# bplaut/PyTorch-VAE

Measured on AMD Instinct MI355X. Metric: train images/sec (node) VanillaVAE 64×64 bs=64 at 1/2/4/8 GPU; ELBO match, higher is better.
Workload: dtype bf16; 1 GPU; VanillaVAE latent_dim=128 64x64 train step (fwd+ELBO+bwd+Adam); per_gpu_batch=64, global_batch=64, parallelism=dp1, graph=True, comm=none

## Files before the change

pytorch-vae_amd/csrc/vae_cgemm.hpp:

```cpp
#pragma once
#include "vae_igemm.hpp"

namespace vae {

template <int BM, int BN> struct CgWaves {
  static constexpr int WN = BN >= 2 * BM ? 4 : (BM >= 2 * BN ? 1 : 2);
  static constexpr int WM = 4 / WN;
  static constexpr int TM = BM / WM / 16, TN = BN / WN / 16;
  static_assert(TM >= 1 && TN >= 1, "wave tile below 16x16");
};

template <int XA>
__device__ __forceinline__ uint4 cg_xform(const uint32_t (&w)[4], const uint32_t (&y)[4], const Tab& t, int ch,
                                          float slope) {
  if constexpr (XA == VAE_X_NONE) {
    return uint4{w[0], w[1], w[2], w[3]};
  } else {
    uint4 o;
    uint32_t* op = reinterpret_cast<uint32_t*>(&o);
    f32x2 ab[4], bb[4], cb[4];
    if constexpr (XA != VAE_X_ACT) {
      const f32x4 a0 = tab4(t.a, ch), a1 = tab4(t.a, ch + 4);
      ab[0] = f32x2{a0[0], a0[1]}; ab[1] = f32x2{a0[2], a0[3]}; ab[2] = f32x2{a1[0], a1[1]}; ab[3] = f32x2{a1[2], a1[3]};
      {
// ... 40 lines not shown
template <int LOADS> constexpr int wg_stages() {
  return 20 / LOADS < 2 ? 2 : (20 / LOADS > 8 ? 8 : 20 / LOADS);
}

template <int BM, int BN, int BK, int NBUF = 2> struct CgSmem {
  static constexpr int LDK = BK + 8;
  static constexpr int LOOP = NBUF * (BM + BN) * LDK * 2;
  static constexpr int EPI = BM * (BN + 4) * 4;
  static constexpr int BYTES = LOOP > EPI ? LOOP : EPI;
};

template <int BM, int BN, int XA> constexpr int cg_waves_per_eu() {
  return (BM >= 128 && BN >= 128) ? 2 : ((BM == 64 && BN == 32 && XA == VAE_X_BN_DY) ? 3 : 1);
}

template <int BM, int BN, int BK, int AM, int XA, int EM, int OR>
__device__ __forceinline__ void cgemm_body(const GemmParams& p, const int bid, char* smem) {
  using WG = CgWaves<BM, BN>;
  constexpr int TM = WG::TM, TN = WG::TN, WTM = TM * 16, WTN = TN * 16;
  constexpr int LDK = CgSmem<BM, BN, BK>::LDK;
  constexpr int KC = BK / 8;
  constexpr int RPP = 256 / KC;
  constexpr int APT = (BM + RPP - 1) / RPP, BPT = (BN + RPP - 1) / RPP;
  constexpr bool DY = XA == VAE_X_BN_DY;
  constexpr int NSF = OR == 3 ? cg_ring_deep(APT * (DY ? 2 : 1) + BPT) : cg_stages<APT * (DY ? 2 : 1) + BPT>();
  constexpr int NS = OR == 2 ? (NSF < 2 ? NSF : 2) : NSF;
  constexpr int NBUF = OR == 2 ? 1 : 2;
  constexpr bool ABN = XA == VAE_X_BN_ACT || XA == VAE_X_BN_DY;
  static_assert(BM % RPP == 0 || BM < RPP, "A tile rows");
  static_assert(BN % RPP == 0 || BN < RPP, "B tile rows");

  extern __shared__ float tabs[];
  __bf16* As = reinterpret_cast<__bf16*>(smem);
  __bf16* Bs = As + NBUF * BM * LDK;

#ifdef VAE_PROBE
  unsigned long long clk[4] = {0, 0, 0, 0};
  const unsigned long long wall0 = threadIdx.x == 0 ? wall_clock64() : 0;
#endif
  PROBE_MARK(0);
  const int tid = threadIdx.x, lane = tid & 63;
  const int wave = __builtin_amdgcn_readfirstlane(tid >> 6);
  const int wm = wave / WG::WN, wn = wave % WG::WN;
  const int gm = (p.M + BM - 1) / BM, gn = (p.N + BN - 1) / BN, gz = p.nphase * p.ksplit;
  int tile;
  {
    const int nb = gm * gn * gz, b = bid;
    const int q = nb >> 3, r = nb & 7, x = b & 7, loc = b >> 3;
    tile = x * q + min(x, r) + loc;
  }
  int tn, tz, tmi;
  if (p.m_fast) { tmi = tile % gm; tz = (tile / gm) % gz; tn = tile / (gm * gz); }
  else { tn = tile % gn; tz = (tile / gn) % gz; tmi = tile / (gn * gz); }
  const int m0 = tmi * BM, n0 = tn * BN;
  const int phase = (p.nphase > 1) ? (int)(tz / p.ksplit) : 0;
  const int ks = tz - phase * p.ksplit;
  const bool first_block = tile == 0;

  const PhaseInfo pq = make_phase(p, phase);
  const int Kp = AM == A_CONVT ? pq.nth * pq.ntw * p.gc : p.K;
  const int ktiles = (Kp + BK - 1) / BK;
  const int kper = (ktiles + p.ksplit - 1) / p.ksplit;
  const int kt0 = ks * kper;
  const int kt1 = min(ktiles, kt0 + kper);
  const int kend = min(Kp, kt1 * BK);

  const int kc = tid % KC, r0 = tid / KC;
  const Src<__bf16> sa = make_src<__bf16>(p.a_ptr, p.a_bytes, p.a_xf);
  const rsrc_t rb = make_rsrc(p.b_ptr, p.b_bytes);
  RowOperand<__bf16, AM, true> ar[APT];
  int bbase[BPT];
  bool bok[BPT];
#pragma unroll
  for (int i = 0; i < APT; ++i) ar[i].init(p, m0 + r0 + i * RPP, p.M, phase, p.a_ld);
#pragma unroll
  for (int i = 0; i < BPT; ++i) {
    const int n = n0 + r0 + i * RPP;
    bok[i] = n < p.N && r0 + i * RPP < BN;
    bbase[i] = n * p.b_ld;
// ... 32 lines not shown
      const uint32_t off = (bok[i] && t.kin) ? (uint32_t)(bbase[i] + boff) * 2u : kOOB;
      bload<16>(rb, off, st.b[i]);
    }
  };

  const int ca = tab_stride(p.a_xf.channels), ce = tab_stride(p.epi_xf.channels);
  const Tab ta{tabs, tabs + ca, tabs + 2 * ca, nullptr, nullptr};
  float* tq = tabs + (ABN ? 3 * ca : 0);
  const Tab te{tq, tq + ce, nullptr, tq + 2 * ce, tq + 3 * ce};

  constexpr int TCH = 2;
  float tva[3][TCH], tve[4][TCH];
  const bool a_tab = ABN && p.a_xf.table != nullptr && p.a_xf.channels <= 256 * TCH;
  const bool e_tab = EM == E_BNBWD && p.epi_xf.kind == VAE_X_BN_ACT && p.epi_xf.table != nullptr &&
                     p.epi_xf.channels <= 256 * TCH;
  if (a_tab) {
    const int C = p.a_xf.channels;
#pragma unroll
    for (int j = 0; j < TCH; ++j) {
      const int ch = min(tid + 256 * j, C - 1);
#pragma unroll
      for (int q = 0; q < (DY ? 3 : 2); ++q) tva[q][j] = p.a_xf.table[q * C + ch];
    }
  }
  if (e_tab) {
    const int C = p.epi_xf.channels;
#pragma unroll
    for (int j = 0; j < TCH; ++j) {
      const int ch = min(tid + 256 * j, C - 1);
#pragma unroll
      for (int q = 0; q < 4; ++q) tve[q][j] = p.epi_xf.table[q * C + ch];
    }
  }
  TabPre<DY ? 4 : 2> pa;
  TabPre<2> pe;
  const bool a_pre = ABN && !a_tab && tab_pre_ok<XA>(p.a_xf);
  const bool e_pre = EM == E_BNBWD && !e_tab && tab_pre_ok<VAE_X_BN_ACT>(p.epi_xf);
  if (a_pre) tab_pre_load(p.a_xf, pa);
  if (e_pre) tab_pre_load(p.epi_xf, pe);
  Stage ring[NS];
#pragma unroll
  for (int u = 0; u < NS; ++u) {
    if (!OR || kt0 + u < kt1) issue(kt0 + u, ring[u]);
  }
  constexpr int EC = BN / 8, ERS = 256 / EC;
  constexpr int EPT = (BM + ERS - 1) / ERS;
  const int ec = tid % EC, er0 = tid / EC;
  const int col = n0 + ec * 8;
  const bool col_ok = col < p.N;
  uint32_t aux[EPT][4], res[EPT][4];
  int obase[EPT];
  bool rok[EPT];
  float bias[8];
  const bool has_res = p.residual != nullptr;
  constexpr bool EARLY = EPT <= 2 && cg_waves_per_eu<BM, BN, XA>() < 3;
  auto epi_loads = [&]() {
    const rsrc_t raux = epi_aux_rsrc<EM>(p);
    const rsrc_t rres = epi_res_rsrc<EM>(p);
    const bool loads = p.slab == nullptr;
#pragma unroll
    for (int i = 0; i < EPT; ++i) {
      const int rl = er0 + i * ERS, row = m0 + rl;
      rok[i] = rl < BM && row < p.M && col_ok;
      obase[i] = out_row_base(p, phase, rok[i] ? row : 0) + col;
      const uint32_t off = (rok[i] && loads) ? (uint32_t)obase[i] * 2u : kOOB;
      bload<16>(raux, off, aux[i]);
      if (EM == E_BNBWD && has_res) bload<16>(rres, off, res[i]);
      else res[i][0] = res[i][1] = res[i][2] = res[i][3] = 0u;
    }
#pragma unroll
    for (int e = 0; e < 8; ++e) bias[e] = 0.f;
    if (EM == E_STORE && p.bias && col_ok && loads) {
#pragma unroll
      for (int e = 0; e < 8; ++e) bias[e] = p.bias[col + e];
    }
  };
  if constexpr (EARLY) epi_loads();
  if (a_tab) {
    const int C = p.a_xf.channels;
#pragma unroll
    for (int j = 0; j < TCH; ++j) {
      const int ch = tid + 256 * j;
      if (ch < C) {
        ta.a[ch] = tva[0][j]; ta.b[ch] = tva[1][j];
        if (DY) ta.c[ch] = tva[2][j];
      }
    }
  } else if constexpr (ABN) {
    tab_fill_pre(p.a_xf, pa, a_pre, ta, false, first_block, reinterpret_cast<float*>(smem));
  }
  if constexpr (ABN) {
    if (tid < 8) { const int z = tab_pad(p.a_xf.channels) + tid; ta.a[z] = 0.f; ta.b[z] = 0.f; ta.c[z] = 0.f; }
  }
  if (e_tab) {
    const int C = p.epi_xf.channels;
#pragma unroll
    for (int j = 0; j < TCH; ++j) {
      const int ch = tid + 256 * j;
      if (ch < C) { te.a[ch] = tve[0][j]; te.b[ch] = tve[1][j]; te.p[ch] = tve[2][j]; te.q[ch] = tve[3][j]; }
    }
  } else if constexpr (EM == E_BNBWD) {
    tab_fill_pre(p.epi_xf, pe, e_pre, te, true, false, reinterpret_cast<float*>(smem));
  }
  __syncthreads();
  PROBE_MARK(1);

  f32x4 acc[TM][TN];
#pragma unroll
  for (int i = 0; i < TM; ++i)
#pragma unroll
    for (int j = 0; j < TN; ++j) acc[i][j] = f32x4{0.f, 0.f, 0.f, 0.f};

  auto store = [&](int buf, const Stage& st) {
    __bf16* ad = As + buf * BM * LDK + r0 * LDK + kc * 8;
#pragma unroll
    for (int i = 0; i < APT; ++i) {
      if (r0 + i * RPP < BM) {
// ... 20 lines not shown
      bf16x8 af[TM], bfr[TN];
#pragma unroll
      for (int i = 0; i < TM; ++i) af[i] = *reinterpret_cast<const bf16x8*>(a + i * 16 * LDK + 32 * kk);
#pragma unroll
      for (int j = 0; j < TN; ++j) bfr[j] = *reinterpret_cast<const bf16x8*>(b + j * 16 * LDK + 32 * kk);
#pragma unroll
      for (int i = 0; i < TM; ++i)
#pragma unroll
        for (int j = 0; j < TN; ++j) acc[i][j] = __builtin_amdgcn_mfma_f32_16x16x32_bf16(af[i], bfr[j], acc[i][j], 0, 0, 0);
    }
  };

  if constexpr (OR != 0) {
#pragma unroll
    for (int u = 0; u < NS; ++u) {
      if (kt0 + u < kt1) {
        if (NBUF == 1 && u > 0) __syncthreads();
        store(u & (NBUF - 1), ring[u]);
        __syncthreads();
        compute(u & (NBUF - 1));
      }
    }
  } else {
    int buf = 0;
    for (int kb = kt0; kb < kt1; kb += NS) {
#pragma unroll
      for (int u = 0; u < NS; ++u) {
        const bool live = kb + u < kt1;
        if (live) store(buf, ring[u]);
        __syncthreads();
        issue(kb + u + NS, ring[u]);
        if (live) compute(buf);
        buf ^= 1;
      }
    }
  }
  PROBE_MARK(2);
#ifdef VAE_PROBE
  struct ProbeEnd {
    unsigned long long* pr; unsigned long long* clk; unsigned long long w0;
    __device__ ~ProbeEnd() { PROBE_MARK(3); probe_write(pr, clk, w0); }
  } probe_end{p.probe, clk, wall0};
#endif

  __shared__ float fpart[CgWaves<BM, BN>::WM][2][BN];
  const bool frag_sums = EM == E_STORE && p.sum != nullptr && p.slab == nullptr;
  if (frag_sums) {
#pragma unroll
    for (int j = 0; j < TN; ++j) {
      float a1 = 0.f, a2 = 0.f;
#pragma unroll
      for (int i = 0; i < TM; ++i)
#pragma unroll
        for (int e = 0; e < 4; ++e) { a1 += acc[i][j][e]; a2 = fmaf(acc[i][j][e], acc[i][j][e], a2); }
      a1 += __shfl_xor(a1, 16); a2 += __shfl_xor(a2, 16);
      a1 += __shfl_xor(a1, 32); a2 += __shfl_xor(a2, 32);
      if (lane < 16) { fpart[wm][0][wn * WTN + j * 16 + lane] = a1; fpart[wm][1][wn * WTN + j * 16 + lane] = a2; }
    }
  }
  __syncthreads();
  float* Cs = reinterpret_cast<float*>(smem);
  constexpr int LDC = BN + 4;
  {
    const int rq = wm * WTM + 4 * (lane >> 4), cq = wn * WTN + (lane & 15);
#pragma unroll
    for (int i = 0; i < TM; ++i)
#pragma unroll
      for (int j = 0; j < TN; ++j)
#pragma unroll
        for (int e = 0; e < 4; ++e) Cs[(rq + i * 16 + e) * LDC + cq + j * 16] = acc[i][j][e];
  }
  __syncthreads();
  if (p.slab) {
    float* sl = p.slab + ((long)(phase * p.ksplit + ks) * p.M) * p.N;
#pragma unroll
    for (int i = 0; i < EPT; ++i) {
      const int rl = er0 + i * ERS, row = m0 + rl;
      if (rl < BM && row < p.M && col_ok) {
// ... 55 lines not shown
        }
        o[e] = g;
      }
    }
    uint32_t* pp = reinterpret_cast<uint32_t*>(&pk[i]);
#pragma unroll
    for (int e = 0; e < 4; ++e) {
      bf16x2 h;
      h[0] = (__bf16)o[2 * e];
      h[1] = (__bf16)o[2 * e + 1];
      pp[e] = *reinterpret_cast<uint32_t*>(&h);
    }
  }
  if (frag_sums) {
    for (int c = tid; c < BN; c += 256) {
      if (n0 + c < p.N) {
        float t1 = 0.f, t2 = 0.f;
#pragma unroll
        for (int w = 0; w < CgWaves<BM, BN>::WM; ++w) { t1 += fpart[w][0][c]; t2 += fpart[w][1][c]; }
        epi_flush_sums<EM>(p, bid, n0 + c, t1, t2);
      }
    }
  } else if (EM == E_BNBWD && epi_wants_sums<EM>(p)) {
    float* part = Cs;
#pragma unroll
    for (int m = EC; m < 64; m <<= 1) {
#pragma unroll
      for (int e = 0; e < 8; ++e) {
        s1[e] += __shfl_xor(s1[e], m);
        s2[e] += __shfl_xor(s2[e], m);
      }
    }
    __syncthreads();
    if (lane < EC) {
#pragma unroll
      for (int e = 0; e < 8; ++e) {
        part[(wave * 2) * BN + ec * 8 + e] = s1[e];
        part[(wave * 2 + 1) * BN + ec * 8 + e] = s2[e];
      }
    }
    __syncthreads();
    for (int c = tid; c < BN; c += 256) {
      if (n0 + c < p.N) {
        const float t1 = (part[0 * BN + c] + part[2 * BN + c]) + (part[4 * BN + c] + part[6 * BN + c]);
        const float t2 = (part[1 * BN + c] + part[3 * BN + c]) + (part[5 * BN + c] + part[7 * BN + c]);
        epi_flush_sums<EM>(p, bid, n0 + c, t1, t2);
      }
    }
  }
  __bf16* out = static_cast<__bf16*>(p.out);
#pragma unroll
  for (int i = 0; i < EPT; ++i)
    if (rok[i]) *reinterpret_cast<uint4*>(out + obase[i]) = pk[i];
}

template <int BM, int BN, int BK, int OR> constexpr int cg_nbuf() { return OR == 2 ? 1 : 2; }

template <int BM, int BN, int BK, int AM, int XA, int EM, int OR>
__global__ void __launch_bounds__(256) __attribute__((amdgpu_waves_per_eu(cg_waves_per_eu<BM, BN, XA>())))
cgemm_kernel(const GemmParams p) {
  kernarg_prefetch<sizeof(GemmParams)>();
  __shared__ __attribute__((aligned(16))) char smem[CgSmem<BM, BN, BK, cg_nbuf<BM, BN, BK, OR>()>::BYTES];
  cgemm_body<BM, BN, BK, AM, XA, EM, OR>(p, (int)blockIdx.x, smem);
}

}
```

pytorch-vae_amd/csrc/vae_common.hpp:

```cpp
#pragma once
#include <hip/hip_runtime.h>
#include <stdint.h>
#include <string.h>

#include "vaehip.h"

typedef float f32x4 __attribute__((ext_vector_type(4)));
typedef float f32x2 __attribute__((ext_vector_type(2)));
typedef __bf16 bf16x8 __attribute__((ext_vector_type(8)));
typedef __bf16 bf16x4 __attribute__((ext_vector_type(4)));
typedef __bf16 bf16x2 __attribute__((ext_vector_type(2)));

namespace vae {

void set_error(const char* fmt, ...);
int fail(int code, const char* fmt, ...);
int check_launch(const char* what);
int bn_finalize_launch(const vae_bn_args* a, hipStream_t stream);
constexpr int kRouteDeclined = 0x7fff0001;

inline int grid_for(long n, int per_block = 256, int max_blocks = 2048) {
  long b = (n + per_block - 1) / per_block;
  if (b < 1) b = 1;
  return (int)(b > max_blocks ? max_blocks : b);
// ... 310 lines not shown
__host__ __device__ inline int tab_stride(int c) { return tab_pad(c) + 8; }

__host__ __device__ inline bool bn_fast_ok(const vae_xform& x) {
  const int C = x.channels, R = x.reps > 1 ? x.reps : 1;
  if (C <= 0 || C > 512 || R * C > 1024 || (x.reps > 1 && x.rstride < C)) return false;
  return C <= 256 ? (256 % C == 0) : (C % 256 == 0);
}

template <int NS>
struct TabPre {
  float v[NS][4];
  float g, be, sh;
};

template <int NS>
__device__ __forceinline__ void tab_pre_load(const vae_xform& x, TabPre<NS>& q) {
  const int C = x.channels, R = x.reps > 1 ? x.reps : 1, tid = threadIdx.x;
  const long rs = x.reps > 1 ? x.rstride : 0;
  const int total = R * C;
  const float* arr[4] = {x.sum, x.sumsq, x.dgamma, x.dbeta};
#pragma unroll
  for (int k = 0; k < 4; ++k) {
    const int f = tid + 256 * k;
    const bool ok = f < total;
    const int r = ok ? f / C : 0, c = ok ? f - r * C : 0;
    const long o = (long)r * rs + c;
#pragma unroll
    for (int a = 0; a < NS; ++a) q.v[a][k] = ok ? arr[a][o] : 0.f;
  }
  const int ch = tid < C ? tid : C - 1;
  q.g = x.gamma[ch];
  q.be = x.beta[ch];
  q.sh = x.shift ? x.shift[ch] : 0.0f;
}

template <int NS>
__device__ __forceinline__ void tab_pre_finish(const vae_xform& x, const TabPre<NS>& q, Tab t, bool epi,
                                               bool update_running, float* scr) {
  const int C = x.channels, R = x.reps > 1 ? x.reps : 1, tid = threadIdx.x;
  float tot[2][4];
#pragma unroll
  for (int j = 0; j < 2; ++j)
#pragma unroll
    for (int a = 0; a < 4; ++a) tot[j][a] = 0.f;
  int nch = 1;
  if (C <= 256) {
#pragma unroll
    for (int a = 0; a < NS; ++a) scr[a * 256 + tid] = (q.v[a][0] + q.v[a][1]) + (q.v[a][2] + q.v[a][3]);
    __syncthreads();
    if (tid < C) {
#pragma unroll
      for (int a = 0; a < NS; ++a) {
        float acc = 0.f;
        for (int j = tid; j < 256; j += C) acc += scr[a * 256 + j];
        tot[0][a] = acc;
      }
    }
    __syncthreads();
    nch = tid < C ? 1 : 0;
  } else {
    const int per = C / 256;
#pragma unroll
    for (int j = 0; j < 2; ++j)
#pragma unroll
      for (int a = 0; a < NS; ++a) {
        float acc = 0.f;
#pragma unroll
        for (int k = 0; k < 4; ++k) acc += ((k % per) == j && k / per < R) ? q.v[a][k] : 0.f;
        tot[j][a] = acc;
      }
    nch = per;
  }
#pragma unroll
  for (int j = 0; j < 2; ++j) {
    if (j >= nch) break;
    const int ch = C <= 256 ? tid : tid + 256 * j;
    const float g = j == 0 ? q.g : x.gamma[ch];
    const float be = j == 0 ? q.be : x.beta[ch];
    const float sh = j == 0 ? q.sh : (x.shift ? x.shift[ch] : 0.0f);
    const BnMom mo = bn_mom(tot[j][0], tot[j][1], sh, x);
    if (x.kind == VAE_X_BN_ACT) {
      const BnFwd f = bn_fwd(mo, g);
      t.a[ch] = f.a;
      t.b[ch] = f.b(be);
      if (epi) { t.p[ch] = f.p; t.q[ch] = f.q; }
      if (update_running && x.running_mean) {
// ... 1 lines not shown
        const float unb = x.count > 1.f ? mo.var * x.count / (x.count - 1.f) : mo.var;
        x.running_mean[ch] = (1.f - m) * x.running_mean[ch] + m * mo.mean;
        x.running_var[ch] = (1.f - m) * x.running_var[ch] + m * unb;
      }
    } else {
      const float inv_m = 1.0f / x.count;
      const float A = g * mo.invstd;
      const float mg = tot[j][3] * inv_m, mgx = tot[j][2] * inv_m;
      t.a[ch] = A;
      t.b[ch] = -A * mo.invstd * mgx;
      t.c[ch] = -A * (mg - mo.mean * mo.invstd * mgx);
    }
  }
}

__device__ __forceinline__ void tab_build(const vae_xform& x, Tab t, bool epi, bool update_running, float* scr) {
  if (x.kind == VAE_X_BN_DY) {
    TabPre<4> q;
    tab_pre_load(x, q);
    tab_pre_finish(x, q, t, epi, update_running, scr);
  } else {
    TabPre<2> q;
    tab_pre_load(x, q);
    tab_pre_finish(x, q, t, epi, update_running, scr);
  }
}

__device__ __forceinline__ void tab_build(const vae_xform& x, Tab t, bool epi, bool update_running) {
  __shared__ float scr[4 * 256];
  tab_build(x, t, epi, update_running, scr);
}

constexpr int kSwapT = 64;
__host__ __device__ inline int swap_tiles(const vae_swap_desc& d) {
  return ((d.a + kSwapT - 1) / kSwapT) * ((d.b + kSwapT - 1) / kSwapT) * d.rs;
}
__device__ __forceinline__ void swap_tile(const vae_swap_desc& d, int blk, float (*t)[kSwapT + 1]) {
  const int nb = (d.b + kSwapT - 1) / kSwapT, na = (d.a + kSwapT - 1) / kSwapT;
  const int bt = blk % nb; blk /= nb;
// ... 47 lines not shown
```

pytorch-vae_amd/csrc/vae_conv_bwd_data.hip:

```cpp
#include "vae_launch.hpp"
#include "vae_wgrad.hpp"
#include "vae_c3.hpp"

using namespace vae;

extern "C" int vae_conv2d_bwd_data(const vae_conv_args* a, void* stream) {
  const char* what = "conv2d_bwd_data";
  if (int rc = check_geom(a, what)) return rc;
  if (!a->dy || !a->wt || !a->dx) return fail(VAE_E_BADARG, "conv2d_bwd_data: null tensor");
  if (!xf_ok(a->dy_xf, "conv2d_bwd_data.dy") || !epi_ok(a->dx_epi, "conv2d_bwd_data.epi")) return VAE_E_BADARG;
  if (a->x_nchw_f32) return fail(VAE_E_UNSUPPORTED, "conv2d_bwd_data: no gradient for the NCHW image input");
  const int S = a->stride;
  if (a->h % S || a->w % S || a->h / S != a->p || a->w / S != a->q)
    return fail(VAE_E_BADSHAPE, "conv2d_bwd_data: needs h == p*stride (got h=%d p=%d S=%d)", a->h, a->p, S);
  hipStream_t st = (hipStream_t)stream;
  const bool tile = a->dtype == VAE_BF16 && a->wt_t && a->dy_xf.kind == VAE_X_NONE &&
                    (a->dx_epi.kind == VAE_X_NONE || a->dx_epi.kind == VAE_X_ACT) && !a->dx_dgamma && !a->bn_finalize &&
                    a->split_k <= 0;
  if (tile && pointwise(a) && p1_shape_ok((long)a->n * a->h * a->w, a->k, a->c)) {
    P1Args c;
    memset(&c, 0, sizeof(c));
    c.a = a->dy; c.b = a->wt_t; c.out = a->dx; c.residual = a->residual;
    if (a->dx_epi.kind == VAE_X_ACT) { c.aux = a->dx_epi.aux; c.aux_slope = a->dx_epi.slope; }
    c.M = (long)a->n * a->h * a->w; c.C = a->k; c.N = a->c;
    return p1_launch(c, st);
  }
  if (tile && c3_shape_ok(a->n, a->p, a->q, a->h, a->w, a->r, a->stride, a->pad, a->k, a->c)) {
    C3Args c;
    memset(&c, 0, sizeof(c));
    c.a = a->dy; c.b = a->wt_t; c.flip = 1; c.out = a->dx; c.residual = a->residual;
    if (a->dx_epi.kind == VAE_X_ACT) { c.aux = a->dx_epi.aux; c.aux_slope = a->dx_epi.slope; }
    c.n = a->n; c.C = a->k; c.N = a->c;
    return c3_launch(c, st);
// ... 38 lines not shown
```

pytorch-vae_amd/csrc/vae_conv_fwd.hip:

```cpp
#include "vae_launch.hpp"
#include "vae_wgrad.hpp"
#include "vae_c3.hpp"

using namespace vae;

extern "C" int vae_conv2d_fwd(const vae_conv_args* a, void* stream) {
  if (int rc = check_geom(a, "conv2d_fwd")) return rc;
  if (!a->x || !a->wt || !a->y) return fail(VAE_E_BADARG, "conv2d_fwd: null tensor");
  if (!xf_ok(a->x_xf, "conv2d_fwd.x")) return VAE_E_BADARG;
  hipStream_t st = (hipStream_t)stream;
  const bool tile = a->dtype == VAE_BF16 && !a->x_nchw_f32 && (a->x_xf.kind == VAE_X_NONE || a->x_xf.kind == VAE_X_ACT) &&
                    !a->y_sum && !a->y_sumsq && !a->bn_finalize && a->split_k <= 0;
  if (tile && pointwise(a) && p1_shape_ok((long)a->n * a->p * a->q, a->c, a->k) &&
      (a->residual_xf.kind == VAE_X_NONE || a->residual_xf.kind == VAE_X_ACT)) {
    P1Args c;
    memset(&c, 0, sizeof(c));
    c.a = a->x; c.a_act = a->x_xf.kind == VAE_X_ACT; c.a_slope = a->x_xf.slope;
    c.b = a->wt; c.out = a->y; c.bias = a->bias;
    c.residual = a->residual; c.res_act = a->residual && a->residual_xf.kind == VAE_X_ACT; c.res_slope = a->residual_xf.slope;
    c.M = (long)a->n * a->p * a->q; c.C = a->c; c.N = a->k;
    return p1_launch(c, st);
  }
  if (tile && c3_shape_ok(a->n, a->h, a->w, a->p, a->q, a->r, a->stride, a->pad, a->c, a->k) && !a->residual) {
    C3Args c;
    memset(&c, 0, sizeof(c));
    c.a = a->x; c.a_act = a->x_xf.kind == VAE_X_ACT; c.a_slope = a->x_xf.slope;
    c.b = a->wt; c.flip = 0; c.out = a->y; c.bias = a->bias;
// ... 13 lines not shown
```

pytorch-vae_amd/csrc/vae_igemm.hpp:

```cpp
#pragma once
#include "vae_common.hpp"

namespace vae {

enum AMode { A_CONV = 0, A_CONVT = 1, A_DENSE = 2, A_KM = 3 };
enum BMode { B_NK = 0, B_KN = 1, B_GATHER = 2 };
enum EMode { E_STORE = 0, E_BNBWD = 1, E_ACC = 2, E_REPARAM = 3 };

constexpr int MAXC = 4096;
constexpr int NTHREADS = 256;

template <class T> constexpr int bk_of() { return sizeof(T) == 2 ? 64 : 32; }

struct FastDiv {
  uint32_t d, mul, shr;
  __device__ __forceinline__ uint32_t div(uint32_t n) const { return (__umulhi(n, mul) + n) >> shr; }
};

inline FastDiv make_fastdiv(uint32_t d) {
  FastDiv f;
  f.d = d < 1 ? 1 : d;
  uint32_t l = 0;
  while ((1ull << l) < f.d) ++l;
  f.shr = l;
// ... 69 lines not shown
  q.ntw = q.pw ? p.ntap_w[1] : p.ntap_w[0];
  q.fdw = q.pw ? p.fd_ntw[1] : p.fd_ntw[0];
  q.dh = q.ph ? p.tap_d[1] : p.tap_d[0];
  q.dw = q.pw ? p.tap_d[1] : p.tap_d[0];
  return q;
}

__device__ __forceinline__ void tab_zero_slot(const vae_xform& x, Tab t) {
  if (threadIdx.x < 8) {
    const int z = tab_pad(x.channels) + threadIdx.x;
    t.a[z] = 0.f; t.b[z] = 0.f;
    if (x.kind == VAE_X_BN_DY) t.c[z] = 0.f;
  }
}

__device__ __forceinline__ void tab_fill(const vae_xform& x, Tab t, bool epi, bool update_running, float* scr) {
  if (x.kind != VAE_X_BN_ACT && x.kind != VAE_X_BN_DY) return;
  tab_zero_slot(x, t);
  if (x.table) {
    const int C = x.channels;
    const bool dy = x.kind == VAE_X_BN_DY;
    const int nt = blockDim.x;
    for (int c0 = threadIdx.x; c0 < C; c0 += 4 * nt) {
      float v[4][4];
#pragma unroll
      for (int u = 0; u < 4; ++u) {
        const int ch = c0 + u * nt, cc = ch < C ? ch : C - 1;
        v[u][0] = x.table[cc];
        v[u][1] = x.table[C + cc];
        v[u][2] = (dy || epi) ? x.table[2 * C + cc] : 0.f;
        v[u][3] = (!dy && epi) ? x.table[3 * C + cc] : 0.f;
      }
#pragma unroll
      for (int u = 0; u < 4; ++u) {
        const int ch = c0 + u * nt;
        if (ch >= C) break;
        t.a[ch] = v[u][0]; t.b[ch] = v[u][1];
        if (dy) t.c[ch] = v[u][2];
        else if (epi) { t.p[ch] = v[u][2]; t.q[ch] = v[u][3]; }
      }
    }
    return;
  }
  if (blockDim.x == 256 && bn_fast_ok(x)) {
    tab_build(x, t, epi, update_running, scr);
    return;
  }
  for (int ch = threadIdx.x; ch < x.channels; ch += blockDim.x) {
    BnMom mo;
    bn_moments(x, ch, mo.mean, mo.invstd, mo.var);
    const float g = x.gamma[ch];
    if (x.kind == VAE_X_BN_ACT) {
      const BnFwd f = bn_fwd(mo, g);
      t.a[ch] = f.a;
      t.b[ch] = f.b(x.beta[ch]);
      if (epi) { t.p[ch] = f.p; t.q[ch] = f.q; }
      if (update_running && x.running_mean) {
        const float unb = bn_unbiased(mo, x);
        x.running_mean[ch] = bn_momentum(x, x.running_mean[ch], mo.mean);
        x.running_var[ch] = bn_momentum(x, x.running_var[ch], unb);
      }
    } else {
      const float inv_m = 1.0f / x.count;
      const float A = g * mo.invstd;
      const float mg = rsum(x.dbeta, x, ch) * inv_m;
      const float mgx = rsum(x.dgamma, x, ch) * inv_m;
      t.a[ch] = A;
      t.b[ch] = -A * mo.invstd * mgx;
      t.c[ch] = -A * (mg - mo.mean * mo.invstd * mgx);
    }
  }
}

__device__ __forceinline__ void tab_fill(const vae_xform& x, Tab t, bool epi, bool update_running) {
  __shared__ float scr[4 * 256];
  tab_fill(x, t, epi, update_running, scr);
}

template <int KIND>
__device__ __forceinline__ bool tab_pre_ok(const vae_xform& x) {
  return x.kind == KIND && !x.table && blockDim.x == 256 && bn_fast_ok(x);
}
template <int NS>
__device__ __forceinline__ void tab_fill_pre(const vae_xform& x, const TabPre<NS>& q, bool pre, Tab t, bool epi,
                                             bool update_running, float* scr) {
  if (!pre) { tab_fill(x, t, epi, update_running, scr); return; }
  tab_zero_slot(x, t);
  tab_pre_finish(x, q, t, epi, update_running, scr);
}

__host__ __device__ inline int tab_floats(const vae_xform& x, bool epi) {
  if (x.kind != VAE_X_BN_ACT && x.kind != VAE_X_BN_DY) return 0;
  return (epi ? 4 : 3) * tab_stride(x.channels);
}

constexpr uint32_t kOOB = 0x80000000u;
typedef __amdgpu_buffer_rsrc_t rsrc_t;

__device__ __forceinline__ rsrc_t make_rsrc(const void* ptr, uint32_t bytes) {
  return __builtin_amdgcn_make_buffer_rsrc(const_cast<void*>(ptr), (short)0, (int)bytes, 0x00020000);
}

template <int NB>
// ... 1014 lines not shown
```

pytorch-vae_amd/csrc/vae_launch.hpp:

```cpp
#pragma once
#include "vae_fgemm.hpp"
#include "vae_cgemm.hpp"
#include "vae_bgemm.hpp"
#include "vae_gemm_desc.hpp"
#include <stdlib.h>

#ifdef VAE_PROBE
extern "C" unsigned long long* vae_probe_buffer(void);
#endif

namespace vae {
namespace {

constexpr int kCUs = 256;
constexpr int kTargetBlocks = 512;
constexpr long kLdsBytes = 160 * 1024;

inline long cg_table_bytes(const GemmParams& p, int em) {
  const int k = p.a_xf.kind;
  return 4l * (((k == VAE_X_BN_ACT || k == VAE_X_BN_DY) ? 3 * tab_stride(p.a_xf.channels) : 0) +
               (em == E_BNBWD ? 4 * tab_stride(p.epi_xf.channels) : 0));
}
inline long cg_static_bytes(int bm, int bn) {
  const int bk = bm >= 128 ? 64 : 128;
// ... 292 lines not shown
  p.ksplit = split;
  p.slab = split > 1 ? static_cast<float*>(ws) : nullptr;
  const dim3 grid((p.M + BM - 1) / BM, (p.N + BN - 1) / BN, p.nphase * p.ksplit);
  const size_t lds = (size_t)(tab_floats(p.a_xf, false) + (EM == E_BNBWD ? tab_floats(p.epi_xf, true) : 0)) * 4;
  VAE_LAUNCH((fgemm_kernel<T, TA, BM, BN, AM, EM, DYA>), grid, dim3(256), lds, st, p);
  int rc = check_launch("fgemm");
  if (rc) return rc;
  if (p.slab) return launch_finalize<T, EM>(p, st);
  return VAE_OK;
}

template <int AM, int BMD, int EM, bool DYA, bool DYB, bool A_F32 = false, bool B_F32 = false>
inline int launch(int dtype, bool a_f32, bool b_f32, GemmParams p, int split_req, void* ws, long ws_bytes,
                  hipStream_t st) {
  if (p.M <= 0 || p.N <= 0) return VAE_OK;
  finish_divs(p);
  if constexpr (BMD == B_NK && AM != A_KM && EM != E_ACC) {
    if (!a_f32 && !b_f32 && split_req <= 0 && !p.det && fgemm_ok<AM, BMD, EM>(p)) {
      if (dtype == VAE_F32) return launch_fgemm<float, float, AM, EM, DYA>(p, ws, ws_bytes, st);
      if (dtype == VAE_BF16) return launch_fgemm<__bf16, __bf16, AM, EM, DYA>(p, ws, ws_bytes, st);
    }
  }
  const Tile t = pick_tile(p.M, p.N, p.nphase);
  const int bk = dtype == VAE_F32 ? 32 : 64;
  const int ktiles = (phase_kmax(p, AM) + bk - 1) / bk;
  const long blocks = (long)((p.M + t.bm - 1) / t.bm) * ((p.N + t.bn - 1) / t.bn) * p.nphase;
  if (p.det && dtype != VAE_F32) return fail(VAE_E_UNSUPPORTED, "deterministic reductions need dtype VAE_F32");
  const bool slab = EM != E_ACC || p.det;
  int split = split_req > 0 ? split_req : pick_split(blocks, ktiles);
  if (EM == E_ACC && p.det && split_req <= 0) {
// ... 172 lines not shown
#define VAE_CG_CASE(BM_, BN_) \
  if (t.bm == BM_ && t.bn == BN_) { \
    const unsigned nb = (unsigned)(((p.M + BM_ - 1) / BM_) * ((p.N + BN_ - 1) / BN_) * p.nphase * p.ksplit); \
    VAE_LAUNCH((cgemm_kernel<BM_, BN_, cg_bk<BM_, BN_>(), AM, XA, EM, OR>), dim3(nb), dim3(256), lds, st, p); \
    return; \
  }
  VAE_CG_CASE(128, 128)
  VAE_CG_CASE(128, 32)
  VAE_CG_CASE(64, 64)
  VAE_CG_CASE(64, 32)
  VAE_CG_CASE(32, 64)
  VAE_CG_CASE(32, 32)
#undef VAE_CG_CASE
}

template <int AM, int EM>
inline int cg_launch(GemmParams p, int split_req, void* ws, long ws_bytes, hipStream_t st) {
  if (p.M <= 0 || p.N <= 0) return VAE_OK;
  finish_divs(p);
  const long ob = out_elems(p) * 2;
  if (int rc = set_extents(p, "cgemm", a_elems<AM>(p) * 2, (long)p.N * p.b_ld * 2, ob, ob, "")) return rc;
  if (split_req <= 0 && bgemm_ok(p, AM, EM)) {
    const int rc = bgemm_launch(p, AM, EM, ws, ws_bytes, st);
    if (rc != kRouteDeclined) return rc;
  }
  const CgTile t = cg_pick(p.M, p.N, p.nphase, cg_table_bytes(p, EM),
                           p.a_xf.kind == VAE_X_BN_ACT || p.a_xf.kind == VAE_X_BN_DY);
  const int bk = t.bm >= 128 ? 64 : 128;
  p.m_fast = (long)p.b_bytes > (long)p.a_bytes ? 1 : 0;
  const int ktiles = (phase_kmax(p, AM) + bk - 1) / bk;
  const long blocks = tile_blocks(p.M, p.N, p.nphase, Tile{t.bm, t.bn});
  int split = split_req > 0 ? split_req : 1;
  if (split_req <= 0 && blocks < (long)kCgSplitWg * kCUs && ktiles >= 4) {
    split = (int)((2 * (long)kCgSplitWg * kCUs + blocks - 1) / blocks);
    if (split > ktiles / 2) split = ktiles / 2;
  }
  if (int rc = split_fits(&split, split_req, p, ws, ws_bytes, "cgemm split-K")) return rc;
  p.ksplit = split < 1 ? 1 : split;
  p.slab = p.ksplit > 1 ? static_cast<float*>(ws) : nullptr;
  const int kps = (ktiles + p.ksplit - 1) / p.ksplit;
  const bool dy = p.a_xf.kind == VAE_X_BN_DY;
  const int KCt = bk / 8, RPPt = 256 / KCt;
  const int loads = ((t.bm + RPPt - 1) / RPPt) * (dy ? 2 : 1) + (t.bn + RPPt - 1) / RPPt;
  const int ns = cg_ring(loads);
  const bool one = kps <= ns;
  const bool deep = EM == E_STORE && !one && kps <= cg_ring_deep(loads) && blocks * p.ksplit <= 2l * kCUs;
#define VAE_CG_XA(XA_) (deep ? cg_launch_tile<AM, XA_, EM, (EM == E_STORE ? 3 : 0)>(p, t, st) \
                        : !one ? cg_launch_tile<AM, XA_, EM, 0>(p, t, st) \
                              : kps <= 2 ? cg_launch_tile<AM, XA_, EM, 2>(p, t, st) : cg_launch_tile<AM, XA_, EM, 1>(p, t, st))
  switch (p.a_xf.kind) {
    case VAE_X_NONE: VAE_CG_XA(VAE_X_NONE); break;
    case VAE_X_ACT: VAE_CG_XA(VAE_X_ACT); break;
    case VAE_X_BN_ACT:
      if constexpr (EM == E_STORE) VAE_CG_XA(VAE_X_BN_ACT);
      break;
    case VAE_X_BN_DY:
      if constexpr (EM == E_BNBWD) VAE_CG_XA(VAE_X_BN_DY);
      break;
  }
#undef VAE_CG_XA
  int rc = check_launch("cgemm");
  if (rc) return rc;
  if (p.slab) return launch_finalize<__bf16, EM>(p, st);
  return VAE_OK;
// ... 35 lines not shown
```

Baseline: 142,400 images/s.

## Add intra-workgroup wave teams that split K for small 32x32 conv-GEMM tiles

Adds an NT template parameter to the conv-GEMM kernel, so a 512- or 1024-thread workgroup runs 2 or 4 teams of 256 threads. Each team covers a slice of the K loop with its own operand ring in LDS. Non-lead teams hand their accumulators to team 0 through LDS, and only team 0 builds the BN tables and runs the epilogue. The goal is more parallelism for small-grid GEMMs without split-K workspace passes and a finalize kernel. Teams start automatically only for a 32x32 tile, no split-K, at most one workgroup per CU and enough LDS, or on request via a negative split_k. The cost is bigger workgroups, an extra LDS reduction and more barriers.

```diff
diff --git a/pytorch-vae_amd/csrc/vae_cgemm.hpp b/pytorch-vae_amd/csrc/vae_cgemm.hpp
--- a/pytorch-vae_amd/csrc/vae_cgemm.hpp
+++ b/pytorch-vae_amd/csrc/vae_cgemm.hpp
@@ -78,8 +78,15 @@
   return (BM >= 128 && BN >= 128) ? 2 : ((BM == 64 && BN == 32 && XA == VAE_X_BN_DY) ? 3 : 1);
 }
 
-template <int BM, int BN, int BK, int AM, int XA, int EM, int OR>
+template <int BM, int BN, int NT> struct CgTeams {
+  static constexpr int RED = (NT - 1) * BM * BN * 4;
+  static constexpr int RED_OFF = (CgSmem<BM, BN, 128>::EPI + 255) & ~255;
+};
+
+template <int BM, int BN, int BK, int AM, int XA, int EM, int OR, int NT = 1>
 __device__ __forceinline__ void cgemm_body(const GemmParams& p, const int bid, char* smem) {
+  static_assert(NT == 1 || NT == 2 || NT == 4, "team count");
+  static_assert(NT == 1 || OR == 0 || OR == 1, "teams: ring or one-round kernels only");
   using WG = CgWaves<BM, BN>;
   constexpr int TM = WG::TM, TN = WG::TN, WTM = TM * 16, WTN = TN * 16;
   constexpr int LDK = CgSmem<BM, BN, BK>::LDK;
@@ -95,7 +102,9 @@
   static_assert(BN % RPP == 0 || BN < RPP, "B tile rows");
 
   extern __shared__ float tabs[];
-  __bf16* As = reinterpret_cast<__bf16*>(smem);
+  const int team = NT == 1 ? 0 : __builtin_amdgcn_readfirstlane((int)(threadIdx.x >> 8));
+  const bool lead = NT == 1 || team == 0;
+  __bf16* As = reinterpret_cast<__bf16*>(smem + (NT == 1 ? 0 : team * CgSmem<BM, BN, BK, NBUF>::LOOP));
   __bf16* Bs = As + NBUF * BM * LDK;
 
 #ifdef VAE_PROBE
@@ -103,7 +112,7 @@
   const unsigned long long wall0 = threadIdx.x == 0 ? wall_clock64() : 0;
 #endif
   PROBE_MARK(0);
-  const int tid = threadIdx.x, lane = tid & 63;
+  const int tid = NT == 1 ? (int)threadIdx.x : (int)(threadIdx.x & 255), lane = tid & 63;
   const int wave = __builtin_amdgcn_readfirstlane(tid >> 6);
   const int wm = wave / WG::WN, wn = wave % WG::WN;
   const int gm = (p.M + BM - 1) / BM, gn = (p.N + BN - 1) / BN, gz = p.nphase * p.ksplit;
@@ -125,8 +134,15 @@
   const int Kp = AM == A_CONVT ? pq.nth * pq.ntw * p.gc : p.K;
   const int ktiles = (Kp + BK - 1) / BK;
   const int kper = (ktiles + p.ksplit - 1) / p.ksplit;
-  const int kt0 = ks * kper;
-  const int kt1 = min(ktiles, kt0 + kper);
+  int kt0 = ks * kper;
+  int kt1 = min(ktiles, kt0 + kper);
+  int nmax = kt1 - kt0;
+  if constexpr (NT > 1) {
+    const int n = kt1 - kt0, q = n / NT, r = n % NT;
+    nmax = q + (r > 0 ? 1 : 0);
+    kt0 += team * q + min(team, r);
+    kt1 = kt0 + q + (team < r ? 1 : 0);
+  }
   const int kend = min(Kp, kt1 * BK);
 
   const int kc = tid % KC, r0 = tid / KC;
@@ -189,7 +205,7 @@
   const bool a_tab = ABN && p.a_xf.table != nullptr && p.a_xf.channels <= 256 * TCH;
   const bool e_tab = EM == E_BNBWD && p.epi_xf.kind == VAE_X_BN_ACT && p.epi_xf.table != nullptr &&
                      p.epi_xf.channels <= 256 * TCH;
-  if (a_tab) {
+  if (a_tab && lead) {
     const int C = p.a_xf.channels;
 #pragma unroll
     for (int j = 0; j < TCH; ++j) {
@@ -198,7 +214,7 @@
       for (int q = 0; q < (DY ? 3 : 2); ++q) tva[q][j] = p.a_xf.table[q * C + ch];
     }
   }
-  if (e_tab) {
+  if (e_tab && lead) {
     const int C = p.epi_xf.channels;
 #pragma unroll
     for (int j = 0; j < TCH; ++j) {
@@ -209,10 +225,10 @@
   }
   TabPre<DY ? 4 : 2> pa;
   TabPre<2> pe;
-  const bool a_pre = ABN && !a_tab && tab_pre_ok<XA>(p.a_xf);
-  const bool e_pre = EM == E_BNBWD && !e_tab && tab_pre_ok<VAE_X_BN_ACT>(p.epi_xf);
-  if (a_pre) tab_pre_load(p.a_xf, pa);
-  if (e_pre) tab_pre_load(p.epi_xf, pe);
+  const bool a_pre = ABN && !a_tab && tab_pre_ok<XA>(p.a_xf, 256);
+  const bool e_pre = EM == E_BNBWD && !e_tab && tab_pre_ok<VAE_X_BN_ACT>(p.epi_xf, 256);
+  if (a_pre) tab_pre_load(p.a_xf, pa, lead);
+  if (e_pre) tab_pre_load(p.epi_xf, pe, lead);
   Stage ring[NS];
 #pragma unroll
   for (int u = 0; u < NS; ++u) {
@@ -232,7 +248,7 @@
   auto epi_loads = [&]() {
     const rsrc_t raux = epi_aux_rsrc<EM>(p);
     const rsrc_t rres = epi_res_rsrc<EM>(p);
-    const bool loads = p.slab == nullptr;
+    const bool loads = p.slab == nullptr && lead;
 #pragma unroll
     for (int i = 0; i < EPT; ++i) {
       const int rl = er0 + i * ERS, row = m0 + rl;
@@ -256,26 +272,26 @@
 #pragma unroll
     for (int j = 0; j < TCH; ++j) {
       const int ch = tid + 256 * j;
-      if (ch < C) {
+      if (ch < C && lead) {
         ta.a[ch] = tva[0][j]; ta.b[ch] = tva[1][j];
         if (DY) ta.c[ch] = tva[2][j];
       }
     }
   } else if constexpr (ABN) {
-    tab_fill_pre(p.a_xf, pa, a_pre, ta, false, first_block, reinterpret_cast<float*>(smem));
+    tab_fill_pre(p.a_xf, pa, a_pre, ta, false, first_block, reinterpret_cast<float*>(smem), lead, 256);
   }
   if constexpr (ABN) {
-    if (tid < 8) { const int z = tab_pad(p.a_xf.channels) + tid; ta.a[z] = 0.f; ta.b[z] = 0.f; ta.c[z] = 0.f; }
+    if (tid < 8 && lead) { const int z = tab_pad(p.a_xf.channels) + tid; ta.a[z] = 0.f; ta.b[z] = 0.f; ta.c[z] = 0.f; }
   }
   if (e_tab) {
     const int C = p.epi_xf.channels;
 #pragma unroll
     for (int j = 0; j < TCH; ++j) {
       const int ch = tid + 256 * j;
-      if (ch < C) { te.a[ch] = tve[0][j]; te.b[ch] = tve[1][j]; te.p[ch] = tve[2][j]; te.q[ch] = tve[3][j]; }
+      if (ch < C && lead) { te.a[ch] = tve[0][j]; te.b[ch] = tve[1][j]; te.p[ch] = tve[2][j]; te.q[ch] = tve[3][j]; }
     }
   } else if constexpr (EM == E_BNBWD) {
-    tab_fill_pre(p.epi_xf, pe, e_pre, te, true, false, reinterpret_cast<float*>(smem));
+    tab_fill_pre(p.epi_xf, pe, e_pre, te, true, false, reinterpret_cast<float*>(smem), lead, 256);
   }
   __syncthreads();
   PROBE_MARK(1);
@@ -326,16 +342,17 @@
   if constexpr (OR != 0) {
 #pragma unroll
     for (int u = 0; u < NS; ++u) {
-      if (kt0 + u < kt1) {
+      if (u < nmax) {
+        const bool live = NT == 1 || kt0 + u < kt1;
         if (NBUF == 1 && u > 0) __syncthreads();
-        store(u & (NBUF - 1), ring[u]);
+        if (live) store(u & (NBUF - 1), ring[u]);
         __syncthreads();
-        compute(u & (NBUF - 1));
+        if (live) compute(u & (NBUF - 1));
       }
     }
   } else {
     int buf = 0;
-    for (int kb = kt0; kb < kt1; kb += NS) {
+    for (int kb = kt0; kb < kt0 + nmax; kb += NS) {
 #pragma unroll
       for (int u = 0; u < NS; ++u) {
         const bool live = kb + u < kt1;
@@ -357,7 +374,26 @@
 
   __shared__ float fpart[CgWaves<BM, BN>::WM][2][BN];
   const bool frag_sums = EM == E_STORE && p.sum != nullptr && p.slab == nullptr;
-  if (frag_sums) {
+  if constexpr (NT > 1) {
+    f32x4* red = reinterpret_cast<f32x4*>(smem + CgTeams<BM, BN, NT>::RED_OFF);
+    __syncthreads();
+    if (!lead) {
+#pragma unroll
+      for (int i = 0; i < TM; ++i)
+#pragma unroll
+        for (int j = 0; j < TN; ++j) red[(((team - 1) * TM + i) * TN + j) * 256 + tid] = acc[i][j];
+    }
+    __syncthreads();
+    if (lead) {
+#pragma unroll
+      for (int t = 1; t < NT; ++t)
+#pragma unroll
+        for (int i = 0; i < TM; ++i)
+#pragma unroll
+          for (int j = 0; j < TN; ++j) acc[i][j] += red[(((t - 1) * TM + i) * TN + j) * 256 + tid];
+    }
+  }
+  if (frag_sums && lead) {
 #pragma unroll
     for (int j = 0; j < TN; ++j) {
       float a1 = 0.f, a2 = 0.f;
@@ -373,7 +409,7 @@
   __syncthreads();
   float* Cs = reinterpret_cast<float*>(smem);
   constexpr int LDC = BN + 4;
-  {
+  if (lead) {
     const int rq = wm * WTM + 4 * (lane >> 4), cq = wn * WTN + (lane & 15);
 #pragma unroll
     for (int i = 0; i < TM; ++i)
@@ -459,7 +495,7 @@
   }
   if (frag_sums) {
     for (int c = tid; c < BN; c += 256) {
-      if (n0 + c < p.N) {
+      if (n0 + c < p.N && lead) {
         float t1 = 0.f, t2 = 0.f;
 #pragma unroll
         for (int w = 0; w < CgWaves<BM, BN>::WM; ++w) { t1 += fpart[w][0][c]; t2 += fpart[w][1][c]; }
@@ -477,7 +513,7 @@
       }
     }
     __syncthreads();
-    if (lane < EC) {
+    if (lane < EC && lead) {
 #pragma unroll
       for (int e = 0; e < 8; ++e) {
         part[(wave * 2) * BN + ec * 8 + e] = s1[e];
@@ -486,7 +522,7 @@
     }
     __syncthreads();
     for (int c = tid; c < BN; c += 256) {
-      if (n0 + c < p.N) {
+      if (n0 + c < p.N && lead) {
         const float t1 = (part[0 * BN + c] + part[2 * BN + c]) + (part[4 * BN + c] + part[6 * BN + c]);
         const float t2 = (part[1 * BN + c] + part[3 * BN + c]) + (part[5 * BN + c] + part[7 * BN + c]);
         epi_flush_sums<EM>(p, bid, n0 + c, t1, t2);
@@ -496,17 +532,24 @@
   __bf16* out = static_cast<__bf16*>(p.out);
 #pragma unroll
   for (int i = 0; i < EPT; ++i)
-    if (rok[i]) *reinterpret_cast<uint4*>(out + obase[i]) = pk[i];
+    if (rok[i] && lead) *reinterpret_cast<uint4*>(out + obase[i]) = pk[i];
 }
 
 template <int BM, int BN, int BK, int OR> constexpr int cg_nbuf() { return OR == 2 ? 1 : 2; }
 
-template <int BM, int BN, int BK, int AM, int XA, int EM, int OR>
-__global__ void __launch_bounds__(256) __attribute__((amdgpu_waves_per_eu(cg_waves_per_eu<BM, BN, XA>())))
+template <int BM, int BN, int BK, int OR, int NT> constexpr int cg_smem_bytes() {
+  using S = CgSmem<BM, BN, BK, cg_nbuf<BM, BN, BK, OR>()>;
+  return NT == 1 ? S::BYTES : NT * S::LOOP;
+}
+
+template <int BM, int BN, int BK, int AM, int XA, int EM, int OR, int NT = 1>
+__global__ void __launch_bounds__(256 * NT) __attribute__((amdgpu_waves_per_eu(cg_waves_per_eu<BM, BN, XA>())))
 cgemm_kernel(const GemmParams p) {
   kernarg_prefetch<sizeof(GemmParams)>();
-  __shared__ __attribute__((aligned(16))) char smem[CgSmem<BM, BN, BK, cg_nbuf<BM, BN, BK, OR>()>::BYTES];
-  cgemm_body<BM, BN, BK, AM, XA, EM, OR>(p, (int)blockIdx.x, smem);
-}
-
-}
+  static_assert(NT == 1 || CgTeams<BM, BN, NT>::RED_OFF + CgTeams<BM, BN, NT>::RED <= CgSmem<BM, BN, BK>::LOOP,
+                "the handed-over accumulator tiles fit team 0's operand ring");
+  __shared__ __attribute__((aligned(16))) char smem[cg_smem_bytes<BM, BN, BK, OR, NT>()];
+  cgemm_body<BM, BN, BK, AM, XA, EM, OR, NT>(p, (int)blockIdx.x, smem);
+}
+
+}
diff --git a/pytorch-vae_amd/csrc/vae_common.hpp b/pytorch-vae_amd/csrc/vae_common.hpp
--- a/pytorch-vae_amd/csrc/vae_common.hpp
+++ b/pytorch-vae_amd/csrc/vae_common.hpp
@@ -348,8 +348,16 @@
 };
 
 template <int NS>
-__device__ __forceinline__ void tab_pre_load(const vae_xform& x, TabPre<NS>& q) {
+__device__ __forceinline__ void tab_pre_load(const vae_xform& x, TabPre<NS>& q, bool active = true) {
   const int C = x.channels, R = x.reps > 1 ? x.reps : 1, tid = threadIdx.x;
+  if (!active) {
+#pragma unroll
+    for (int k = 0; k < 4; ++k)
+#pragma unroll
+      for (int a = 0; a < NS; ++a) q.v[a][k] = 0.f;
+    q.g = q.be = q.sh = 0.f;
+    return;
+  }
   const long rs = x.reps > 1 ? x.rstride : 0;
   const int total = R * C;
   const float* arr[4] = {x.sum, x.sumsq, x.dgamma, x.dbeta};
@@ -370,7 +378,7 @@
 
 template <int NS>
 __device__ __forceinline__ void tab_pre_finish(const vae_xform& x, const TabPre<NS>& q, Tab t, bool epi,
-                                               bool update_running, float* scr) {
+                                               bool update_running, float* scr, bool active = true) {
   const int C = x.channels, R = x.reps > 1 ? x.reps : 1, tid = threadIdx.x;
   float tot[2][4];
 #pragma unroll
@@ -380,9 +388,10 @@
   int nch = 1;
   if (C <= 256) {
 #pragma unroll
-    for (int a = 0; a < NS; ++a) scr[a * 256 + tid] = (q.v[a][0] + q.v[a][1]) + (q.v[a][2] + q.v[a][3]);
+    for (int a = 0; a < NS; ++a)
+      if (active) scr[a * 256 + tid] = (q.v[a][0] + q.v[a][1]) + (q.v[a][2] + q.v[a][3]);
     __syncthreads();
-    if (tid < C) {
+    if (active && tid < C) {
 #pragma unroll
       for (int a = 0; a < NS; ++a) {
         float acc = 0.f;
@@ -391,7 +400,7 @@
       }
     }
     __syncthreads();
-    nch = tid < C ? 1 : 0;
+    nch = (active && tid < C) ? 1 : 0;
   } else {
     const int per = C / 256;
 #pragma unroll
@@ -403,7 +412,7 @@
         for (int k = 0; k < 4; ++k) acc += ((k % per) == j && k / per < R) ? q.v[a][k] : 0.f;
         tot[j][a] = acc;
       }
-    nch = per;
+    nch = active ? per : 0;
   }
 #pragma unroll
   for (int j = 0; j < 2; ++j) {
@@ -435,15 +444,16 @@
   }
 }
 
-__device__ __forceinline__ void tab_build(const vae_xform& x, Tab t, bool epi, bool update_running, float* scr) {
+__device__ __forceinline__ void tab_build(const vae_xform& x, Tab t, bool epi, bool update_running, float* scr,
+                                          bool active = true) {
   if (x.kind == VAE_X_BN_DY) {
     TabPre<4> q;
-    tab_pre_load(x, q);
-    tab_pre_finish(x, q, t, epi, update_running, scr);
+    tab_pre_load(x, q, active);
+    tab_pre_finish(x, q, t, epi, update_running, scr, active);
   } else {
     TabPre<2> q;
-    tab_pre_load(x, q);
-    tab_pre_finish(x, q, t, epi, update_running, scr);
+    tab_pre_load(x, q, active);
+    tab_pre_finish(x, q, t, epi, update_running, scr, active);
   }
 }
 
diff --git a/pytorch-vae_amd/csrc/vae_conv_bwd_data.hip b/pytorch-vae_amd/csrc/vae_conv_bwd_data.hip
--- a/pytorch-vae_amd/csrc/vae_conv_bwd_data.hip
+++ b/pytorch-vae_amd/csrc/vae_conv_bwd_data.hip
@@ -16,7 +16,7 @@
   hipStream_t st = (hipStream_t)stream;
   const bool tile = a->dtype == VAE_BF16 && a->wt_t && a->dy_xf.kind == VAE_X_NONE &&
                     (a->dx_epi.kind == VAE_X_NONE || a->dx_epi.kind == VAE_X_ACT) && !a->dx_dgamma && !a->bn_finalize &&
-                    a->split_k <= 0;
+                    a->split_k == 0;
   if (tile && pointwise(a) && p1_shape_ok((long)a->n * a->h * a->w, a->k, a->c)) {
     P1Args c;
     memset(&c, 0, sizeof(c));
diff --git a/pytorch-vae_amd/csrc/vae_conv_fwd.hip b/pytorch-vae_amd/csrc/vae_conv_fwd.hip
--- a/pytorch-vae_amd/csrc/vae_conv_fwd.hip
+++ b/pytorch-vae_amd/csrc/vae_conv_fwd.hip
@@ -10,7 +10,7 @@
   if (!xf_ok(a->x_xf, "conv2d_fwd.x")) return VAE_E_BADARG;
   hipStream_t st = (hipStream_t)stream;
   const bool tile = a->dtype == VAE_BF16 && !a->x_nchw_f32 && (a->x_xf.kind == VAE_X_NONE || a->x_xf.kind == VAE_X_ACT) &&
-                    !a->y_sum && !a->y_sumsq && !a->bn_finalize && a->split_k <= 0;
+                    !a->y_sum && !a->y_sumsq && !a->bn_finalize && a->split_k == 0;
   if (tile && pointwise(a) && p1_shape_ok((long)a->n * a->p * a->q, a->c, a->k) &&
       (a->residual_xf.kind == VAE_X_NONE || a->residual_xf.kind == VAE_X_ACT)) {
     P1Args c;
diff --git a/pytorch-vae_amd/csrc/vae_igemm.hpp b/pytorch-vae_amd/csrc/vae_igemm.hpp
--- a/pytorch-vae_amd/csrc/vae_igemm.hpp
+++ b/pytorch-vae_amd/csrc/vae_igemm.hpp
@@ -107,13 +107,14 @@
   }
 }
 
-__device__ __forceinline__ void tab_fill(const vae_xform& x, Tab t, bool epi, bool update_running, float* scr) {
+__device__ __forceinline__ void tab_fill(const vae_xform& x, Tab t, bool epi, bool update_running, float* scr,
+                                         bool active, int nt) {
   if (x.kind != VAE_X_BN_ACT && x.kind != VAE_X_BN_DY) return;
-  tab_zero_slot(x, t);
+  if (active) tab_zero_slot(x, t);
   if (x.table) {
+    if (!active) return;
     const int C = x.channels;
     const bool dy = x.kind == VAE_X_BN_DY;
-    const int nt = blockDim.x;
     for (int c0 = threadIdx.x; c0 < C; c0 += 4 * nt) {
       float v[4][4];
 #pragma unroll
@@ -135,11 +136,12 @@
     }
     return;
   }
-  if (blockDim.x == 256 && bn_fast_ok(x)) {
-    tab_build(x, t, epi, update_running, scr);
+  if (nt == 256 && bn_fast_ok(x)) {
+    tab_build(x, t, epi, update_running, scr, active);
     return;
   }
-  for (int ch = threadIdx.x; ch < x.channels; ch += blockDim.x) {
+  if (!active) return;
+  for (int ch = threadIdx.x; ch < x.channels; ch += nt) {
     BnMom mo;
     bn_moments(x, ch, mo.mean, mo.invstd, mo.var);
     const float g = x.gamma[ch];
@@ -165,21 +167,32 @@
   }
 }
 
+__device__ __forceinline__ void tab_fill(const vae_xform& x, Tab t, bool epi, bool update_running, float* scr) {
+  tab_fill(x, t, epi, update_running, scr, true, (int)blockDim.x);
+}
+
 __device__ __forceinline__ void tab_fill(const vae_xform& x, Tab t, bool epi, bool update_running) {
   __shared__ float scr[4 * 256];
   tab_fill(x, t, epi, update_running, scr);
 }
 
 template <int KIND>
-__device__ __forceinline__ bool tab_pre_ok(const vae_xform& x) {
-  return x.kind == KIND && !x.table && blockDim.x == 256 && bn_fast_ok(x);
+__device__ __forceinline__ bool tab_pre_ok(const vae_xform& x, int nt) {
+  return x.kind == KIND && !x.table && nt == 256 && bn_fast_ok(x);
+}
+template <int KIND>
+__device__ __forceinline__ bool tab_pre_ok(const vae_xform& x) { return tab_pre_ok<KIND>(x, (int)blockDim.x); }
+template <int NS>
+__device__ __forceinline__ void tab_fill_pre(const vae_xform& x, const TabPre<NS>& q, bool pre, Tab t, bool epi,
+                                             bool update_running, float* scr, bool active, int nt) {
+  if (!pre) { tab_fill(x, t, epi, update_running, scr, active, nt); return; }
+  if (active) tab_zero_slot(x, t);
+  tab_pre_finish(x, q, t, epi, update_running, scr, active);
 }
 template <int NS>
 __device__ __forceinline__ void tab_fill_pre(const vae_xform& x, const TabPre<NS>& q, bool pre, Tab t, bool epi,
                                              bool update_running, float* scr) {
-  if (!pre) { tab_fill(x, t, epi, update_running, scr); return; }
-  tab_zero_slot(x, t);
-  tab_pre_finish(x, q, t, epi, update_running, scr);
+  tab_fill_pre(x, q, pre, t, epi, update_running, scr, true, (int)blockDim.x);
 }
 
 __host__ __device__ inline int tab_floats(const vae_xform& x, bool epi) {
diff --git a/pytorch-vae_amd/csrc/vae_launch.hpp b/pytorch-vae_amd/csrc/vae_launch.hpp
--- a/pytorch-vae_amd/csrc/vae_launch.hpp
+++ b/pytorch-vae_amd/csrc/vae_launch.hpp
@@ -330,6 +330,8 @@
 inline int launch(int dtype, bool a_f32, bool b_f32, GemmParams p, int split_req, void* ws, long ws_bytes,
                   hipStream_t st) {
   if (p.M <= 0 || p.N <= 0) return VAE_OK;
+  if (split_req < 0)
+    return fail(VAE_E_BADARG, "split_k %d: wave teams exist on the bf16 conv-GEMM path only, which this call does not take", split_req);
   finish_divs(p);
   if constexpr (BMD == B_NK && AM != A_KM && EM != E_ACC) {
     if (!a_f32 && !b_f32 && split_req <= 0 && !p.det && fgemm_ok<AM, BMD, EM>(p)) {
@@ -532,13 +534,28 @@
 #undef VAE_CG_CASE
 }
 
+template <int AM, int EM> constexpr bool cg_team_class() { return true; }
+inline long cg_team_bytes(int nt, long table_bytes) {
+  return (long)nt * CgSmem<32, 32, 128>::LOOP + 2 * 2 * 32 * 4 + 256 + table_bytes;
+}
+
+template <int AM, int XA, int EM, int OR>
+inline void cg_launch_team(const GemmParams& p, int nt, hipStream_t st) {
+  const size_t lds = (size_t)cg_table_bytes(p, EM);
+  const unsigned nb = (unsigned)(((p.M + 31) / 32) * ((p.N + 31) / 32) * p.nphase);
+  if (nt == 4) VAE_LAUNCH((cgemm_kernel<32, 32, 128, AM, XA, EM, OR, 4>), dim3(nb), dim3(1024), lds, st, p);
+  else VAE_LAUNCH((cgemm_kernel<32, 32, 128, AM, XA, EM, OR, 2>), dim3(nb), dim3(512), lds, st, p);
+}
+
 template <int AM, int EM>
 inline int cg_launch(GemmParams p, int split_req, void* ws, long ws_bytes, hipStream_t st) {
   if (p.M <= 0 || p.N <= 0) return VAE_OK;
+  if (split_req < 0 && split_req != -2 && split_req != -4)
+    return fail(VAE_E_BADARG, "cgemm: split_k %d (a negative split_k asks for 2 or 4 wave teams: -2, -4)", split_req);
   finish_divs(p);
   const long ob = out_elems(p) * 2;
   if (int rc = set_extents(p, "cgemm", a_elems<AM>(p) * 2, (long)p.N * p.b_ld * 2, ob, ob, "")) return rc;
-  if (split_req <= 0 && bgemm_ok(p, AM, EM)) {
+  if (split_req == 0 && bgemm_ok(p, AM, EM)) {
     const int rc = bgemm_launch(p, AM, EM, ws, ws_bytes, st);
     if (rc != kRouteDeclined) return rc;
   }
@@ -549,14 +566,27 @@
   const int ktiles = (phase_kmax(p, AM) + bk - 1) / bk;
   const long blocks = tile_blocks(p.M, p.N, p.nphase, Tile{t.bm, t.bn});
   int split = split_req > 0 ? split_req : 1;
-  if (split_req <= 0 && blocks < (long)kCgSplitWg * kCUs && ktiles >= 4) {
+  if (split_req == 0 && blocks < (long)kCgSplitWg * kCUs && ktiles >= 4) {
     split = (int)((2 * (long)kCgSplitWg * kCUs + blocks - 1) / blocks);
     if (split > ktiles / 2) split = ktiles / 2;
   }
   if (int rc = split_fits(&split, split_req, p, ws, ws_bytes, "cgemm split-K")) return rc;
   p.ksplit = split < 1 ? 1 : split;
   p.slab = p.ksplit > 1 ? static_cast<float*>(ws) : nullptr;
-  const int kps = (ktiles + p.ksplit - 1) / p.ksplit;
+  int nt = 1;
+  const bool team_shape = t.bm == 32 && t.bn == 32 && blocks <= kCUs;
+  const long tb = cg_table_bytes(p, EM);
+  if (split_req < 0) {
+    nt = -split_req;
+    if (!team_shape || ktiles < 2 * nt || cg_team_bytes(nt, tb) > kLdsBytes)
+      return fail(VAE_E_BADARG, "cgemm: split_k %d: %d wave teams need a 32x32 tile (planned %dx%d), at most %d workgroups "
+                  "(%ld), at least %d K-steps (%d) and %ld bytes of LDS (%ld)", split_req, nt, t.bm, t.bn, kCUs, blocks,
+                  2 * nt, ktiles, cg_team_bytes(nt, tb), kLdsBytes);
+  } else if (split_req == 0 && p.ksplit == 1 && team_shape && cg_team_class<AM, EM>()) {
+    for (int c = 4; c >= 2 && nt == 1; c >>= 1)
+      if (ktiles >= 2 * c && cg_team_bytes(c, tb) <= kLdsBytes) nt = c;
+  }
+  const int kps = nt > 1 ? (ktiles + nt - 1) / nt : (ktiles + p.ksplit - 1) / p.ksplit;
   const bool dy = p.a_xf.kind == VAE_X_BN_DY;
   const int KCt = bk / 8, RPPt = 256 / KCt;
   const int loads = ((t.bm + RPPt - 1) / RPPt) * (dy ? 2 : 1) + (t.bn + RPPt - 1) / RPPt;
@@ -566,6 +596,21 @@
 #define VAE_CG_XA(XA_) (deep ? cg_launch_tile<AM, XA_, EM, (EM == E_STORE ? 3 : 0)>(p, t, st) \
                         : !one ? cg_launch_tile<AM, XA_, EM, 0>(p, t, st) \
                               : kps <= 2 ? cg_launch_tile<AM, XA_, EM, 2>(p, t, st) : cg_launch_tile<AM, XA_, EM, 1>(p, t, st))
+#define VAE_CG_TEAM(XA_) (one ? cg_launch_team<AM, XA_, EM, 1>(p, nt, st) : cg_launch_team<AM, XA_, EM, 0>(p, nt, st))
+  if (nt > 1) {
+    switch (p.a_xf.kind) {
+      case VAE_X_NONE: VAE_CG_TEAM(VAE_X_NONE); break;
+      case VAE_X_ACT: VAE_CG_TEAM(VAE_X_ACT); break;
+      case VAE_X_BN_ACT:
+        if constexpr (EM == E_STORE) VAE_CG_TEAM(VAE_X_BN_ACT);
+        break;
+      case VAE_X_BN_DY:
+        if constexpr (EM == E_BNBWD) VAE_CG_TEAM(VAE_X_BN_DY);
+        break;
+    }
+    return check_launch("cgemm");
+  }
+#undef VAE_CG_TEAM
   switch (p.a_xf.kind) {
     case VAE_X_NONE: VAE_CG_XA(VAE_X_NONE); break;
     case VAE_X_ACT: VAE_CG_XA(VAE_X_ACT); break;
```

New measurement: 131,100 images/s. 7.9% lower.
